# lixirui142/VidToMe

Measured on AMD Instinct MI355X. Metric: denoising steps/sec, 16-frame 512x512 SD-1.5 chunk, ratio=0.5, higher is better.
Workload: dtype f16 tokens; matching f16-MFMA filter + f32 exact refine (f32-identical indices); attention f16 MFMA with f32 accumulate

## Files before the change

vidtome_amd/build.py:

```python
from __future__ import annotations

import concurrent.futures
import os
import shutil
import subprocess
import sys

HERE = os.path.dirname(os.path.abspath(__file__))
CSRC = os.path.join(HERE, "csrc")
LIBDIR = os.path.join(HERE, "lib")
LIB = os.path.join(LIBDIR, "libvidtome_hip.so")
SOURCES = ["api.hip", "normalize.hip", "match.hip", "match_filter.hip", "sort.hip", "order.hip", "plan.hip", "gather.hip", "attention.hip", "attention16.hip", "attention16g.hip", "ddim.hip", "layernorm.hip", "geglu.hip", "linear.hip", "ff.hip", "lora.hip"]
ARCH = "gfx950"
FLAGS = ["--offload-arch=" + ARCH, "-O3", "-std=c++17", "-fPIC", "-fvisibility=hidden",
         "-ffp-contract=off", "-fno-fast-math", "-Wall", "-Wno-unused-function",
         "-mllvm", "-amdgpu-mfma-vgpr-form=1"]


def hipcc() -> str:
    for cand in (os.environ.get("HIPCC"), shutil.which("hipcc"), "/opt/rocm/bin/hipcc"):
        if cand and os.path.exists(cand):
            return cand
    raise RuntimeError("hipcc not found (need ROCm >= 7.0 for gfx950)")


def _stale(target: str, deps) -> bool:
    if not os.path.exists(target):
        return True
    t = os.path.getmtime(target)
    return any(os.path.getmtime(d) > t for d in deps)


def build(force: bool = False, verbose: bool = False, defines=(), tag: str = "") -> str:
    libdir = os.path.join(LIBDIR, "variants", tag) if tag else LIBDIR
    lib = os.path.join(libdir, "libvidtome_hip.so")
    os.makedirs(libdir, exist_ok=True)
    cc = hipcc()
    headers = [os.path.join(CSRC, "common.h"), os.path.join(CSRC, "ablate.h"), os.path.join(HERE, "..", "include", "vidtome_hip.h")]
    objs, jobs = [], []
    flags = FLAGS + ["-D" + d for d in defines]
    for src in SOURCES:
        s = os.path.join(CSRC, src)
        o = os.path.join(libdir, src.replace(".hip", ".o"))
        objs.append(o)
        if force or _stale(o, [s] + headers):
            jobs.append([cc, *flags, "-c", s, "-o", o])

    def run(cmd):
        if verbose:
            print(" ".join(cmd), flush=True)
        p = subprocess.run(cmd, stdout=subprocess.PIPE, stderr=subprocess.STDOUT, text=True)
        if p.returncode != 0:
            raise RuntimeError("hipcc failed:\n" + " ".join(cmd) + "\n" + p.stdout)
        return p.stdout

    with concurrent.futures.ThreadPoolExecutor(max_workers=min(8, max(1, len(jobs)))) as ex:
        for out in ex.map(run, jobs):
            if verbose and out.strip():
                print(out)
    if force or jobs or _stale(lib, objs):
        run([cc, "--offload-arch=" + ARCH, "-shared", "-fPIC", "-o", lib, *objs])
    return lib


def kernel_resources(obj: str) -> dict:
    import re
    import tempfile
    llvm = os.path.join(os.path.dirname(os.path.dirname(os.path.realpath(hipcc()))), "lib", "llvm", "bin")
    if not os.path.isdir(llvm):
        llvm = "/opt/rocm/lib/llvm/bin"
    with tempfile.TemporaryDirectory() as tmp:
        fat, dev = os.path.join(tmp, "fat.bin"), os.path.join(tmp, "dev.co")
        for cmd in ([os.path.join(llvm, "llvm-objcopy"), "--dump-section", ".hip_fatbin=" + fat, obj],
                    [os.path.join(llvm, "clang-offload-bundler"), "--type=o", "--unbundle", "--input=" + fat, "--output=" + dev,
                     "--targets=hipv4-amdgcn-amd-amdhsa--" + ARCH]):
            p = subprocess.run(cmd, stdout=subprocess.PIPE, stderr=subprocess.STDOUT, text=True)
            if p.returncode != 0:
                raise RuntimeError(" ".join(cmd) + "\n" + p.stdout)
        notes = subprocess.run([os.path.join(llvm, "llvm-readelf"), "--notes", dev], stdout=subprocess.PIPE, text=True,
                               check=True).stdout
    out, cur = {}, None
    for line in notes.splitlines():
        m = re.match(r"\s*\.(name|vgpr_count|sgpr_count|vgpr_spill_count|sgpr_spill_count|private_segment_fixed_size):\s+(\S+)", line)
        if not m:
            continue
        if m.group(1) == "name":
            cur = out.setdefault(m.group(2), {})
        elif cur is not None:
            cur[m.group(1)] = int(m.group(2))
    return {k: v for k, v in out.items() if "vgpr_count" in v}


if __name__ == "__main__":
    argv = sys.argv[1:]
    tag = argv[argv.index("--tag") + 1] if "--tag" in argv else ""
    print(build(force="--force" in argv, verbose=True, defines=[a[2:] for a in argv if a.startswith("-D")], tag=tag))
```

vidtome_amd/csrc/attention16.hip:

```cpp
#include "attention16_parts.h"

#include <algorithm>
#include <type_traits>

namespace {

template <typename T, int D, bool FOLD, int WAVES>
__global__ __launch_bounds__(WAVES * 64, 2) void attention16s_kernel(
    const T *__restrict__ q, int64_t ldq, const T *__restrict__ k, int64_t ldk,
    const T *__restrict__ vt, int64_t ldvt, T *__restrict__ out, int64_t ldo, int64_t H,
    int64_t M, int64_t Mp, int64_t Mk_arg, int64_t Mkp, float scale_log2e, int64_t src_batch, int64_t nqb, int64_t nwhole,
    int nsplit_tail, float *__restrict__ partial_base, int xcd_groups, const int32_t *__restrict__ q_count,
    int64_t split_major_items, const int32_t *__restrict__ k_count, const uint32_t *__restrict__ k_bias, int64_t ldkb,
    const DevPlan *__restrict__ dev_plan) {
    using F = Frag<T>;
    using vec = typename F::vec;
    using elem = typename F::elem;
    static_assert(pv16_for(D) && (D % 16) != 0, "the 16-row O^T path: a head dim with a spare k-slot and a spare O^T row");
    static_assert(!FOLD || (D % 8 == 0 && D % 16 == 8), "key folding needs the spare k-slots of a d % 16 == 8 head");
    constexpr int NQ = 2, KR = 3, VR = 2;
    int64_t tier_item0 = nwhole, tier_wg0 = nwhole, tier_rec0 = 0;
    if (dev_plan != nullptr) {
        nqb = dev_plan->nqb;
        xcd_groups = nqb >= 32 ? xcd_groups : 0;
        int ti = 0;
        while (ti + 1 < dev_plan->ntiers && (int)blockIdx.x >= dev_plan->tier[ti + 1].wg0) ++ti;
        const DevTier tr = dev_plan->tier[ti];
        if ((int64_t)blockIdx.x >= (int64_t)tr.wg0 + (int64_t)tr.items * tr.nsplit) return;
        nwhole = dev_plan->tier[0].items;
        nsplit_tail = tr.nsplit;
        split_major_items = tr.items;
        tier_item0 = tr.item0;
        tier_wg0 = tr.wg0;
        tier_rec0 = tr.rec0;
    }
    constexpr int NT = WAVES * 64, QB = WAVES * QW * NQ, NV = NQ;
    constexpr int DK = (D + 15) / 16, DV16 = (D + 16) / 16, VROWS = vrows_for(D);
    constexpr int BIAS_HI = (D % 16) / 8, BIAS_E = D % 8;
    constexpr int K_STRIDE = DK * 16 + 8;
    constexpr int DCH = D / 8;
    constexpr int K_CHUNKS = KV * DCH, V_CHUNKS = D * (KV / 8);
    constexpr int K_PER_T = (K_CHUNKS + NT - 1) / NT, V_PER_T = (V_CHUNKS + NT - 1) / NT;
    constexpr int SK_TILE = KV * K_STRIDE, SV_TILE = VROWS * VT_STRIDE;
    constexpr int REC = rec16<D>(), NA = DV16 * 8;

    extern __shared__ __attribute__((aligned(16))) char smem[];
    elem *sK = reinterpret_cast<elem *>(smem);
    elem *sV = sK + KR * SK_TILE;

    const int tid = threadIdx.x, lane = tid & 63, wave = tid >> 6;
    const int l31 = lane & 31, hi = lane >> 5;
    const int l15 = lane & 15, g16 = lane >> 4;
    const bool tail_wg = (int64_t)blockIdx.x >= nwhole;
    const int64_t tail_id = (int64_t)blockIdx.x - tier_wg0;
    const int nsplit = tail_wg ? nsplit_tail : 1;
    const int64_t tail_item = split_major_items ? tail_id % split_major_items : tail_id / nsplit;
    const int split = !tail_wg ? 0 : split_major_items ? (int)(tail_id / split_major_items) : (int)(tail_id % nsplit);
    const int64_t lin = item_of(tail_wg ? tier_item0 + tail_item : (int64_t)blockIdx.x, nqb, xcd_groups);
    float *partial = tail_wg ? partial_base + (tier_rec0 + tail_item * nsplit + split) * NV * REC * NT : nullptr;
    const int64_t b = lin / (nqb * H), h = (lin / nqb) % H;
    const int64_t bq = b % src_batch;
    const int64_t qblock0 = (lin % nqb) * QB;
    const int64_t C = H * D;
    int64_t Mk = Mk_arg;
    if constexpr (FOLD) {
        const int64_t kc = k_count[b];
        Mk = kc < Mk_arg ? (kc > 0 ? kc : 1) : Mk_arg;
    }
    if (q_count != nullptr && qblock0 >= (int64_t)q_count[b]) return;

    for (int i = tid; i < KR * KV * (K_STRIDE - D); i += NT) {
        const int row = i / (K_STRIDE - D), c = D + i % (K_STRIDE - D);
        sK[row * K_STRIDE + c] = (elem)(c == D ? 1.0f : 0.0f);
    }
    for (int i = tid; i < VR * (VROWS - D) * VT_STRIDE; i += NT) {
        const int t1 = i / ((VROWS - D) * VT_STRIDE), rem = i % ((VROWS - D) * VT_STRIDE);
        const int row = D + rem / VT_STRIDE, c = rem % VT_STRIDE;
        sV[t1 * SV_TILE + row * VT_STRIDE + c] = (elem)((row == D) ? 1.0f : 0.0f);
    }

    vec qf[NQ][DK];
#pragma unroll
    for (int sub = 0; sub < NQ; ++sub) {
        const int64_t qi = qblock0 + (wave * NQ + sub) * QW + l31;
        const T *qp = q + (bq * Mp + (qi < M ? qi : 0)) * ldq + h * D;
#pragma unroll
        for (int ks = 0; ks < DK; ++ks) {
            const int d0 = ks * 16 + hi * 8;
            uint4 v = make_uint4(0, 0, 0, 0);
            if (d0 < D && qi < M) v = *reinterpret_cast<const uint4 *>(qp + d0);
            qf[sub][ks] = *reinterpret_cast<vec *>(&v);
#pragma unroll
            for (int e = 0; e < 8; ++e) qf[sub][ks][e] = (elem)((float)qf[sub][ks][e] * scale_log2e);
        }
        if constexpr (FOLD) {
            if (hi == BIAS_HI) {
                qf[sub][DK - 1][BIAS_E + 2] = (elem)1.0f;
                qf[sub][DK - 1][BIAS_E + 3] = (elem)1.0f;
            }
        }
    }

    uint32_t kgo[K_PER_T], vgo[V_PER_T];
    int koff[K_PER_T], voff[V_PER_T], krow[K_PER_T], vkey[V_PER_T];
    bool kok[K_PER_T], vok[V_PER_T];
#pragma unroll
    for (int i = 0; i < K_PER_T; ++i) {
        const int c = tid + i * NT;
        kok[i] = c < K_CHUNKS;
        krow[i] = c / DCH;
        kgo[i] = kok[i] ? (uint32_t)(krow[i] * (int)ldk + (c % DCH) * 8) * 2u : 0u;
        koff[i] = krow[i] * K_STRIDE + (c % DCH) * 8;
    }
#pragma unroll
    for (int i = 0; i < V_PER_T; ++i) {
        const int c = tid + i * NT;
        vok[i] = c < V_CHUNKS;
        vkey[i] = (c % (KV / 8)) * 8;
        vgo[i] = vok[i] ? (uint32_t)((c / (KV / 8)) * (int)ldvt + vkey[i]) * 2u : 0u;
        voff[i] = (c / (KV / 8)) * VT_STRIDE + (vkey[i] & ~15) + ((vkey[i] >> 3) & 1) * 4;
    }
    const auto rsrc_k = __builtin_amdgcn_make_buffer_rsrc(const_cast<T *>(k + bq * Mkp * ldk + h * D), 0, 0x7fffffff, 0x00020000);
    const auto rsrc_v = __builtin_amdgcn_make_buffer_rsrc(const_cast<T *>(vt + (b * C + h * D) * ldvt), 0, 0x7fffffff, 0x00020000);
    const uint32_t kstep = (uint32_t)(KV * ldk) * 2u, vstep = (uint32_t)KV * 2u;
    const auto rsrc_b = __builtin_amdgcn_make_buffer_rsrc(const_cast<uint32_t *>(FOLD ? k_bias + b * ldkb : nullptr), 0, 0x7fffffff, 0x00020000);
    uint32_t rbias = 0;
    [[maybe_unused]] const uint32_t bgo = (uint32_t)(tid & (KV - 1)) * 4u;
    auto fetch = [](const auto &rsrc, uint32_t voff_, uint32_t soff_) {
        return __builtin_bit_cast(uint4, __builtin_amdgcn_raw_buffer_load_b128(rsrc, voff_, soff_, 0));
    };

    uint4 rk[K_PER_T], rv[V_PER_T];
    auto issue_k = [&](auto full_tag, int tk) {
        const uint32_t so = (uint32_t)tk * kstep;
        if constexpr (decltype(full_tag)::value) {
#pragma unroll
            for (int i = 0; i < K_PER_T; ++i) rk[i] = fetch(rsrc_k, kgo[i], so);
            if constexpr (FOLD) rbias = __builtin_amdgcn_raw_buffer_load_b32(rsrc_b, bgo, (uint32_t)tk * (uint32_t)KV * 4u, 0);
        } else {
            const int64_t key0 = (int64_t)tk * KV;
#pragma unroll
            for (int i = 0; i < K_PER_T; ++i) {
                uint4 v = make_uint4(0, 0, 0, 0);
                if (kok[i] && key0 + krow[i] < Mk) v = fetch(rsrc_k, kgo[i], so);
                rk[i] = v;
            }
            if constexpr (FOLD) {
                rbias = 0u;
                if (key0 + (tid & (KV - 1)) < Mk) rbias = __builtin_amdgcn_raw_buffer_load_b32(rsrc_b, bgo, (uint32_t)tk * (uint32_t)KV * 4u, 0);
            }
        }
    };
    auto issue_v = [&](auto full_tag, int tv) {
        const uint32_t so = (uint32_t)tv * vstep;
        if constexpr (decltype(full_tag)::value) {
#pragma unroll
            for (int i = 0; i < V_PER_T; ++i) rv[i] = fetch(rsrc_v, vgo[i], so);
        } else {
            const int64_t key0 = (int64_t)tv * KV;
#pragma unroll
            for (int i = 0; i < V_PER_T; ++i) {
                uint4 v = make_uint4(0, 0, 0, 0);
                const int64_t key = key0 + vkey[i];
                if (vok[i] && key < Mk) {
                    v = fetch(rsrc_v, vgo[i], so);
                    mask_keys(v, (int)(Mk - key));
                }
                rv[i] = v;
            }
        }
    };
    auto write_k = [&](int slot) {
        elem *dk = sK + slot * SK_TILE;
        if constexpr (FOLD) {
            if (wave == 0) *reinterpret_cast<uint32_t *>(dk + tid * K_STRIDE + D + 2) = rbias;
        }
#pragma unroll
        for (int i = 0; i < K_PER_T; ++i)
            if (kok[i]) *reinterpret_cast<uint4 *>(dk + koff[i]) = rk[i];
    };
    auto write_v = [&](int slot) {
        elem *dv = sV + slot * SV_TILE;
#pragma unroll
        for (int i = 0; i < V_PER_T; ++i)
            if (vok[i]) {
                uint2 *dst = reinterpret_cast<uint2 *>(dv + voff[i]);
                dst[0] = make_uint2(rv[i].x, rv[i].y);
                dst[2] = make_uint2(rv[i].z, rv[i].w);
            }
    };

    f32x4 o16[NQ][DV16][2];
#pragma unroll
    for (int sub = 0; sub < NQ; ++sub)
#pragma unroll
        for (int dv = 0; dv < DV16; ++dv)
#pragma unroll
            for (int qh = 0; qh < 2; ++qh)
#pragma unroll
                for (int e = 0; e < 4; ++e) o16[sub][dv][qh][e] = 0.0f;
    float m_run[NQ] = {-INFINITY, -INFINITY}, m_bias[NQ] = {0.0f, 0.0f};

    auto load_kf = [&](vec (&kf)[2][DK], int slot) {
#pragma unroll
        for (int kb = 0; kb < 2; ++kb) {
            const elem *kp = sK + slot * SK_TILE + (kb * 32 + l31) * K_STRIDE + hi * 8;
#pragma unroll
            for (int ks = 0; ks < DK; ++ks) kf[kb][ks] = *reinterpret_cast<const vec *>(kp + ks * 16);
        }
    };
    auto qk = [&](f32x16 (&s)[2], const vec (&kf)[2][DK], int sub) {
#pragma unroll
        for (int kb = 0; kb < 2; ++kb) {
#pragma unroll
            for (int r = 0; r < 16; ++r) s[kb][r] = 0.0f;
#pragma unroll
            for (int ks = 0; ks < DK; ++ks) s[kb] = F::mfma(kf[kb][ks], qf[sub][ks], s[kb]);
        }
    };
    auto mask_s = [&](f32x16 (&s)[2], int lim) {
#pragma unroll
        for (int kb = 0; kb < 2; ++kb)
#pragma unroll
            for (int r = 0; r < 16; ++r)
                if (kb * 32 + (r & 3) + 8 * (r >> 2) + 4 * hi >= lim) s[kb][r] = -INFINITY;
    };
    auto rescale = [&](int sub, float alpha) {
#pragma unroll
        for (int qh = 0; qh < 2; ++qh) {
            const float a_ = __shfl(alpha, 16 * qh + l15, 64);
#pragma unroll
            for (int dv = 0; dv < DV16; ++dv)
#pragma unroll
                for (int e = 0; e < 4; ++e) o16[sub][dv][qh][e] *= a_;
        }
    };
    auto raise_shift = [&](f32x16 (&s)[2], int sub) {
        float mt = fmaxf(s[0][0], s[1][0]);
#pragma unroll
        for (int r = 1; r < 16; ++r) mt = fmaxf(fmaxf(mt, s[0][r]), s[1][r]);
        mt = fmaxf(mt, __shfl_xor(mt, 32, 64));
        if (!__all(m_bias[sub] + mt <= m_run[sub] + DEFER_THR)) {
            const float m_new = (float)(elem)(fmaxf(m_run[sub], m_bias[sub] + mt));
            const float alpha = __builtin_amdgcn_exp2f(m_run[sub] - m_new);
            const float delta = m_bias[sub] - m_new;
            m_run[sub] = m_new;
            m_bias[sub] = m_new;
            rescale(sub, alpha);
#pragma unroll
            for (int kb = 0; kb < 2; ++kb)
#pragma unroll
                for (int r = 0; r < 16; ++r) s[kb][r] += delta;
            if (hi == BIAS_HI) qf[sub][DK - 1][BIAS_E] = (elem)(-m_new);
        }
    };
    auto exps = [&](vec (&pf)[4], const f32x16 (&s)[2]) {
#pragma unroll
        for (int st = 0; st < 4; ++st) {
            float p[8];
#pragma unroll
            for (int e = 0; e < 8; ++e) p[e] = __builtin_amdgcn_exp2f(s[st >> 1][8 * (st & 1) + e]);
            F::pack8(pf[st], p);
        }
    };
    auto ptop_of = [&](const vec (&pf)[4]) {
        uint32_t pw[16];
#pragma unroll
        for (int st = 0; st < 4; ++st) {
            const u32x4 w = __builtin_bit_cast(u32x4, pf[st]);
#pragma unroll
            for (int j = 0; j < 4; ++j) pw[4 * st + j] = w[j];
        }
#pragma unroll
        for (int j = 0; j < 5; ++j) pw[j] = F::pmax3(pw[3 * j], pw[3 * j + 1], pw[3 * j + 2]);
        const uint32_t pr = F::pmax3(F::pmax3(pw[0], pw[1], pw[2]), F::pmax3(pw[3], pw[4], pw[15]), pw[15]);
        return max(pr >> 16, pr & 0xffffu);
    };
    auto swaps = [&](vec (&pp)[2][2], const vec (&pf)[4]) {
#pragma unroll
        for (int ks = 0; ks < 2; ++ks) {
            u32x4 x = __builtin_bit_cast(u32x4, pf[2 * ks]), y = __builtin_bit_cast(u32x4, pf[2 * ks + 1]);
#pragma unroll
            for (int w = 0; w < 4; ++w) {
                const auto r = __builtin_amdgcn_permlane16_swap(x[w], y[w], false, false);
                x[w] = r[0];
                y[w] = r[1];
            }
            pp[ks][0] = __builtin_bit_cast(vec, x);
            pp[ks][1] = __builtin_bit_cast(vec, y);
        }
    };
    auto pv = [&](int sub, const vec (&a)[2][DV16], const vec (&pp)[2][2]) {
#pragma unroll
        for (int ks = 0; ks < 2; ++ks)
#pragma unroll
            for (int dv = 0; dv < DV16; ++dv) {
                o16[sub][dv][0] = F::mfma16(a[ks][dv], pp[ks][0], o16[sub][dv][0]);
                o16[sub][dv][1] = F::mfma16(a[ks][dv], pp[ks][1], o16[sub][dv][1]);
            }
    };

    using std::false_type;
    using std::true_type;
    const int ntiles = (int)((Mk + KV - 1) / KV), nfull = (int)(Mk / KV);
    const int tps = (ntiles + nsplit - 1) / nsplit;
    const int tb = split * tps, te = tb + tps < ntiles ? tb + tps : ntiles;
    const int fe = te < nfull ? te : nfull;
    if (tb >= te) {
        if (partial) {
#pragma unroll
            for (int sub = 0; sub < NQ; ++sub) {
                float *pp_ = partial + sub * REC * NT + tid;
#pragma unroll
                for (int r = 0; r < NA; ++r) pp_[r * NT] = 0.0f;
                pp_[NA * NT] = pp_[(NA + 1) * NT] = -INFINITY;
                pp_[(NA + 2) * NT] = 0.0f;
            }
        }
        return;
    }

    if (tb < fe) { issue_k(true_type{}, tb); issue_v(true_type{}, tb); } else { issue_k(false_type{}, tb); issue_v(false_type{}, tb); }
    write_k(0);
    write_v(0);
    if (tb + 1 < te) {
        if (tb + 1 < fe) issue_k(true_type{}, tb + 1); else issue_k(false_type{}, tb + 1);
        write_k(1);
    }
    __syncthreads();

    vec kf[2][DK];
    vec av[2][DV16];
    vec pB[2][2];
    f32x16 sA[2], sB[2];
#pragma unroll
    for (int ks = 0; ks < 2; ++ks) {
#pragma unroll
        for (int dv = 0; dv < DV16; ++dv)
#pragma unroll
            for (int e = 0; e < 8; ++e) av[ks][dv][e] = (elem)0.0f;
#pragma unroll
        for (int qh = 0; qh < 2; ++qh)
#pragma unroll
            for (int e = 0; e < 8; ++e) pB[ks][qh][e] = (elem)0.0f;
    }
    load_kf(kf, 0);
    qk(sA, kf, 0);

    auto iteration = [&](auto fast_tag, int t, int kc, int kn, int kw, int vc) {
        constexpr bool FAST = decltype(fast_tag)::value;
        const int lim = FAST ? KV : (int)(Mk - (int64_t)t * KV);
        if constexpr (FAST) {
            issue_k(true_type{}, t + 2);
            issue_v(true_type{}, t + 1);
        } else {
            if (t + 2 < te) { if (t + 2 < fe) issue_k(true_type{}, t + 2); else issue_k(false_type{}, t + 2); }
            if (t + 1 < te) { if (t + 1 < fe) issue_v(true_type{}, t + 1); else issue_v(false_type{}, t + 1); }
        }
        if constexpr (!FAST) {
            if (lim < KV) mask_s(sA, lim);
        }
        vec pfA[4], ppA[2][2];
        qk(sB, kf, 1);
        pv(1, av, pB);
        exps(pfA, sA);
        const uint32_t topA = ptop_of(pfA);
        if (__any(topA > F::BITS_256 || m_run[0] == -INFINITY)) {
            qk(sA, kf, 0);
            if constexpr (!FAST) {
                if (lim < KV) mask_s(sA, lim);
            }
            raise_shift(sA, 0);
            exps(pfA, sA);
        }
        __builtin_amdgcn_sched_barrier(0);
        if constexpr (!FAST) {
            if (lim < KV) mask_s(sB, lim);
        }
        load_kf(kf, kn);
#pragma unroll
        for (int ks = 0; ks < 2; ++ks)
#pragma unroll
            for (int dv = 0; dv < DV16; ++dv)
                av[ks][dv] = *reinterpret_cast<const vec *>(sV + vc * SV_TILE + (l15 + dv * 16) * VT_STRIDE + (g16 & 1) * 16 +
                                                            (g16 >> 1) * 8 + ks * 32);
        vec pfB[4];
        qk(sA, kf, 0);
        swaps(ppA, pfA);
        pv(0, av, ppA);
        exps(pfB, sB);
        const uint32_t topB = ptop_of(pfB);
        if (__any(topB > F::BITS_256 || m_run[1] == -INFINITY)) {
            vec kfb[2][DK];
            load_kf(kfb, kc);
            qk(sB, kfb, 1);
            if constexpr (!FAST) {
                if (lim < KV) mask_s(sB, lim);
            }
            raise_shift(sB, 1);
            exps(pfB, sB);
        }
        swaps(pB, pfB);
        if constexpr (FAST) {
            write_k(kw);
            write_v(vc ^ 1);
        } else {
            if (t + 2 < te) write_k(kw);
            if (t + 1 < te) write_v(vc ^ 1);
        }
        __syncthreads();
    };

    int t = tb, kc = 0, kn = 1, kw = 2, vc = 0;
    auto rotate = [&]() {
        const int k0 = kc;
        kc = kn;
        kn = kw;
        kw = k0;
        vc ^= 1;
    };
    for (; t + 2 < fe; ++t) {
        iteration(true_type{}, t, kc, kn, kw, vc);
        rotate();
    }
    for (; t < te; ++t) {
        iteration(false_type{}, t, kc, kn, kw, vc);
        rotate();
    }
    pv(1, av, pB);

    if (partial) {
#pragma unroll
        for (int sub = 0; sub < NQ; ++sub) {
            float *pp_ = partial + sub * REC * NT + tid;
#pragma unroll
            for (int r = 0; r < NA; ++r) pp_[r * NT] = o16[sub][r >> 3][(r >> 2) & 1][r & 3];
#pragma unroll
            for (int qh = 0; qh < 2; ++qh) pp_[(NA + qh) * NT] = __shfl(m_run[sub], 16 * qh + l15, 64);
            pp_[(NA + 2) * NT] = 0.0f;
        }
        return;
    }
#pragma unroll
    for (int sub = 0; sub < NQ; ++sub)
        write_output16<T, D>(o16[sub], out, ldo, b, h, qblock0 + (wave * NQ + sub) * QW, M, Mp, lane);
}

template <typename T, int D, bool FOLD, int WAVES>
int launch16(const Args16 &a) {
    constexpr int DK = (D + 15) / 16, NT = WAVES * 64, QB = WAVES * QW * 2, NV = 2;
    constexpr size_t lds = (size_t)(3 * KV * (DK * 16 + 8) + 2 * vrows_for(D) * VT_STRIDE) * 2;
    static_assert(lds <= 64 * 1024, "dynamic LDS beyond 64 KB needs hipFuncSetAttribute");
    const auto kernel = attention16s_kernel<T, D, FOLD, WAVES>;
    const int64_t src_batch = a.B / a.share_groups;
    const size_t rec_bytes = (size_t)NV * rec16<D>() * NT * sizeof(float);
    const float scale_log2e = a.scale * 1.4426950408889634f;
    const int64_t nqb_max = vtm::cdiv(a.M, QB);
    const int xcd_pairs = (a.B * a.h) % 8 == 0 ? (int)(a.B * a.h / 8) : 0;
    const int slots = vtm::device_cus();
    if (a.q_count != nullptr && a.ws != nullptr && a.ws_bytes >= devplan_ws_bytes(slots, rec_bytes) &&
        nqb_max * a.h * a.B >= 2 * slots) {
        DevPlan *plan = reinterpret_cast<DevPlan *>(a.ws);
        float *records = reinterpret_cast<float *>(static_cast<char *>(a.ws) + DEVPLAN_HEADER);
        const int ntiles = (int)vtm::cdiv(a.Mk, KV);
        hipLaunchKernelGGL(attention16_plan_kernel, dim3(1), dim3(64), 0, a.s, a.q_count, (int)a.B, (int)a.h, QB, slots,
                           ntiles, plan);
        const int64_t total = nqb_max * a.h * a.B, tail_max = plan_tail_wgs(slots);
        VTM_REQUIRE(total + tail_max < (1ll << 31) / 16, "vtm_attention: grid too large");
        hipLaunchKernelGGL(kernel, dim3((unsigned)(total + tail_max)), dim3(NT), lds, a.s, (const T *)a.q, a.ldq,
                           (const T *)a.k, a.ldk, (const T *)a.vt, a.ldvt, (T *)a.out, a.ldo, a.h, a.M, a.Mp, a.Mk, a.Mkp,
                           scale_log2e, src_batch, nqb_max, total, 1, records, xcd_pairs, a.q_count, (int64_t)0, a.k_count,
                           a.k_bias, a.ldkb, (const DevPlan *)plan);
        hipLaunchKernelGGL((attention16_combine_kernel<T, D, 2, 1, WAVES>), dim3((unsigned)plan_split_items(slots), (unsigned)NV),
                           dim3(NT), 0, a.s, (const float *)records, (T *)a.out, a.ldo, a.h, a.M, a.Mp, nqb_max, total, 1,
                           xcd_pairs, a.q_count, src_batch, (const DevPlan *)plan);
        return vtm::launch_status("vtm_attention");
    }
    TailPlan p = plan_tail(a.B, a.h, a.M, a.Mk, QB, 1, rec_bytes, a.q_count != nullptr);
    if (p.split_all && (!a.ws || a.ws_bytes < p.ws_bytes)) p = plan_tail(a.B, a.h, a.M, a.Mk, QB, 1, rec_bytes, false);
    if (p.nsplit > 1 && (!a.ws || a.ws_bytes < p.ws_bytes)) {
        p.nsplit = 1;
        p.full = p.total;
        p.split_all = false;
    }
    VTM_REQUIRE(p.total < (1ll << 31) / 16, "vtm_attention: grid too large");
    const int64_t rem = p.total - p.full;
    const int xcd_groups = p.nqb >= 32 ? xcd_pairs : 0;
    hipLaunchKernelGGL(kernel, dim3((unsigned)(p.full + rem * p.nsplit)), dim3(NT), lds,
                       a.s, (const T *)a.q, a.ldq, (const T *)a.k, a.ldk, (const T *)a.vt, a.ldvt, (T *)a.out, a.ldo, a.h, a.M,
                       a.Mp, a.Mk, a.Mkp, scale_log2e, src_batch, p.nqb, p.full, p.nsplit, (float *)a.ws, xcd_groups, a.q_count,
                       p.split_all ? rem : (int64_t)0, a.k_count, a.k_bias, a.ldkb, (const DevPlan *)nullptr);
    if (p.nsplit > 1)
        hipLaunchKernelGGL((attention16_combine_kernel<T, D, 2, 1, WAVES>), dim3((unsigned)rem, (unsigned)NV), dim3(NT), 0, a.s,
                           (const float *)a.ws, (T *)a.out, a.ldo, a.h, a.M, a.Mp, p.nqb, p.full, p.nsplit, xcd_groups,
                           a.q_count, src_batch, (const DevPlan *)nullptr);
    return vtm::launch_status("vtm_attention");
}

template <typename T>
int dispatch16(const Args16 &a) {
    return a.fold ? launch16<T, 40, true, 8>(a) : launch16<T, 40, false, 8>(a);
}

}

namespace vtm_att {

size_t ws_bytes16(int64_t B, int64_t h, int64_t Mq, int64_t Mk, bool bounded) {
    constexpr int WAVES = 8, NT = WAVES * 64;
    const size_t rec = (size_t)2 * rec16<40>() * NT * sizeof(float);
    size_t n = plan_tail(B, h, Mq, Mk, (int64_t)WAVES * QW * 2, 1, rec, bounded).ws_bytes;
    if (bounded) n = std::max(n, devplan_ws_bytes(vtm::device_cus(), rec));
    return n;
}

int attention16(const Args16 &a) {
    if (a.dtype == VTM_F16) return dispatch16<__half>(a);
    if (a.dtype == VTM_BF16) return dispatch16<vtm_bf16>(a);
    return vtm::fail(VTM_EINVAL, "vtm_attention: dtype must be VTM_F16 or VTM_BF16");
}

}
```

Before: 22.08.

## Reorder attention16 inner loop and interleave MFMA with exp/LDS via sched groups

Restructures the two-subtile attention iteration so the PV MFMAs and the next-tile QK MFMAs are issued earlier, with the V and K LDS fragment loads hoisted ahead of the exponent work. It adds sched_group_barrier patterns that interleave each MFMA with transcendental, VALU and LDS-read instructions in the fast path, so the exp work and LDS latency are hidden behind matrix ops. The rare max-raise fallback now reloads the current K tile into a separate register set, because kf already holds the next tile. The build script also tracks all headers as dependencies. Risks are higher register pressure from the extra live fragments, and hand-written schedule groups that may not match the instruction mix the compiler actually emits.

```diff
diff --git a/vidtome_amd/build.py b/vidtome_amd/build.py
--- a/vidtome_amd/build.py
+++ b/vidtome_amd/build.py
@@ -36,7 +36,8 @@
     lib = os.path.join(libdir, "libvidtome_hip.so")
     os.makedirs(libdir, exist_ok=True)
     cc = hipcc()
-    headers = [os.path.join(CSRC, "common.h"), os.path.join(CSRC, "ablate.h"), os.path.join(HERE, "..", "include", "vidtome_hip.h")]
+    headers = [os.path.join(CSRC, h) for h in sorted(os.listdir(CSRC)) if h.endswith(".h")]
+    headers.append(os.path.join(HERE, "..", "include", "vidtome_hip.h"))
     objs, jobs = [], []
     flags = FLAGS + ["-D" + d for d in defines]
     for src in SOURCES:
diff --git a/vidtome_amd/csrc/attention16.hip b/vidtome_amd/csrc/attention16.hip
--- a/vidtome_amd/csrc/attention16.hip
+++ b/vidtome_amd/csrc/attention16.hip
@@ -4,6 +4,20 @@
 #include <type_traits>
 
 namespace {
+
+constexpr int SG_VALU = 0x2, SG_MFMA = 0x8, SG_DS_READ = 0x100, SG_TRANS = 0x400;
+constexpr int SG_NOT_MFMA = 0x7ff & ~SG_MFMA;
+
+template <int NM, int TR, int VA, int DS>
+__device__ __forceinline__ void sched_mfma() {
+#pragma unroll
+    for (int i = 0; i < NM; ++i) {
+        __builtin_amdgcn_sched_group_barrier(SG_MFMA, 1, 0);
+        if constexpr (TR > 0) __builtin_amdgcn_sched_group_barrier(SG_TRANS, TR, 0);
+        if constexpr (VA > 0) __builtin_amdgcn_sched_group_barrier(SG_VALU, VA, 0);
+        if constexpr (DS > 0) __builtin_amdgcn_sched_group_barrier(SG_DS_READ, DS, 0);
+    }
+}
 
 template <typename T, int D, bool FOLD, int WAVES>
 __global__ __launch_bounds__(WAVES * 64, 2) void attention16s_kernel(
@@ -209,6 +223,14 @@
             for (int ks = 0; ks < DK; ++ks) kf[kb][ks] = *reinterpret_cast<const vec *>(kp + ks * 16);
         }
     };
+    auto load_av = [&](vec (&a)[2][DV16], int slot) {
+#pragma unroll
+        for (int ks = 0; ks < 2; ++ks)
+#pragma unroll
+            for (int dv = 0; dv < DV16; ++dv)
+                a[ks][dv] = *reinterpret_cast<const vec *>(sV + slot * SV_TILE + (l15 + dv * 16) * VT_STRIDE + (g16 & 1) * 16 +
+                                                            (g16 >> 1) * 8 + ks * 32);
+    };
     auto qk = [&](f32x16 (&s)[2], const vec (&kf)[2][DK], int sub) {
 #pragma unroll
         for (int kb = 0; kb < 2; ++kb) {
@@ -361,12 +383,22 @@
             if (lim < KV) mask_s(sA, lim);
         }
         vec pfA[4], ppA[2][2];
+        pv(1, av, pB);
+        if constexpr (FAST) __builtin_amdgcn_sched_barrier(SG_NOT_MFMA);
+        load_av(av, vc);
         qk(sB, kf, 1);
-        pv(1, av, pB);
+        load_kf(kf, kn);
         exps(pfA, sA);
         const uint32_t topA = ptop_of(pfA);
+        if constexpr (FAST) {
+            sched_mfma<12, 1, 0, 0>();
+            sched_mfma<6, 2, 2, 1>();
+            __builtin_amdgcn_sched_group_barrier(SG_DS_READ, 2 * DK, 0);
+        }
         if (__any(topA > F::BITS_256 || m_run[0] == -INFINITY)) {
-            qk(sA, kf, 0);
+            vec kfa[2][DK];
+            load_kf(kfa, kc);
+            qk(sA, kfa, 0);
             if constexpr (!FAST) {
                 if (lim < KV) mask_s(sA, lim);
             }
@@ -377,19 +409,17 @@
         if constexpr (!FAST) {
             if (lim < KV) mask_s(sB, lim);
         }
-        load_kf(kf, kn);
-#pragma unroll
-        for (int ks = 0; ks < 2; ++ks)
-#pragma unroll
-            for (int dv = 0; dv < DV16; ++dv)
-                av[ks][dv] = *reinterpret_cast<const vec *>(sV + vc * SV_TILE + (l15 + dv * 16) * VT_STRIDE + (g16 & 1) * 16 +
-                                                            (g16 >> 1) * 8 + ks * 32);
         vec pfB[4];
-        qk(sA, kf, 0);
         swaps(ppA, pfA);
         pv(0, av, ppA);
+        if constexpr (FAST) __builtin_amdgcn_sched_barrier(SG_NOT_MFMA);
+        qk(sA, kf, 0);
         exps(pfB, sB);
         const uint32_t topB = ptop_of(pfB);
+        if constexpr (FAST) {
+            sched_mfma<12, 1, 0, 0>();
+            sched_mfma<6, 2, 0, 0>();
+        }
         if (__any(topB > F::BITS_256 || m_run[1] == -INFINITY)) {
             vec kfb[2][DK];
             load_kf(kfb, kc);
```

After: 22.14 (median of 6 runs). Within noise of the previous version (+0.3%).
